# eth-cscs/COSTA

Hardware: AMD Instinct MI355X
Metric: GB/s device-resident tile pack+transpose+unpack (fp64), % HBM peak (higher is better)
Workload: dtype f64; 1 GPU; pxtran fp64 16384x16384, 256x256 blocks, op T, alpha=1 beta=0, 1x1 grid (BASELINE configs[1]); op=T, parallelism=1 rank(s), one per GPU, RCCL send/recv exchange, m=16384, n=16384, block=256, grid=1x1

## Files before the change

costa_amd/__init__.py:

```python
from __future__ import annotations

import ctypes as C
import os
import struct
from dataclasses import dataclass
from typing import Iterable, Sequence

import numpy as np

__all__ = [
    "CostaError", "lib", "FLOAT", "DOUBLE", "CFLOAT", "CDOUBLE", "INT32", "HALF", "BFLOAT16",
    "FP8_E4M3", "FP8_E5M2", "dtype_code", "element_code",
    "np_dtype", "Layout", "block_cyclic_layout", "custom_layout", "Comm", "transform",
    "transform_batch", "transform_async", "transform_batch_async", "synchronize", "transformer", "copy_and_transform", "execute_tiles", "execute_tiles_mixed",
    "convert_subtile", "TileOp", "TriOp", "TRI_OP_DTYPE", "transform_tri", "transform_tri_async",
    "execute_tiles_tri", "plan_export_tri", "tri_cut", "tri_subtile", "tri_phase_ms",
    "plan_export", "set_profiling", "get_stats", "release_caches", "TILE_OP_DTYPE",
    "ScaledOp", "SCALED_OP_DTYPE", "SCALED_F_ROWS", "transform_scaled", "execute_tiles_scaled",
    "plan_export_scaled", "scaled_subtile", "scaled_items",
]

FLOAT, DOUBLE, CFLOAT, CDOUBLE, INT32 = 0, 1, 2, 3, 4
HALF, BFLOAT16 = 5, 6
_NP = {FLOAT: np.float32, DOUBLE: np.float64, CFLOAT: np.complex64,
       CDOUBLE: np.complex128, INT32: np.int32, HALF: np.float16, BFLOAT16: np.uint16}
_TORCH = {"torch.float32": FLOAT, "torch.float64": DOUBLE, "torch.complex64": CFLOAT,
          "torch.complex128": CDOUBLE, "torch.int32": INT32, "torch.float16": HALF,
          "torch.bfloat16": BFLOAT16}

FP8_E4M3, FP8_E5M2 = 7, 8
_NP_FP8 = {FP8_E4M3: np.uint8, FP8_E5M2: np.uint8}
_TORCH_FP8 = {"torch.float8_e4m3fn": FP8_E4M3, "torch.float8_e5m2": FP8_E5M2}
_FP32_SCALARS = (HALF, BFLOAT16, FP8_E4M3, FP8_E5M2)

TILE_TRANSPOSE, TILE_CONJ, TILE_VEC_SRC, TILE_VEC_DST = 0x1, 0x2, 0x4, 0x8
SCALE_BITCOPY, SCALE_ZERO, SCALE_ALPHA, SCALE_AXPBY = 0, 1, 2, 3

TILE_OP_DTYPE = np.dtype([("src", "<u8"), ("dst", "<u8"), ("nf", "<i4"), ("ns", "<i4"),
                          ("lds", "<i4"), ("ldd", "<i4"), ("flags", "<u4"),
                          ("order", "<u4")])


TRI_LE = 0x40
TRI_OP_DTYPE = np.dtype(TILE_OP_DTYPE.descr + [("diag", "<i4"), ("pad", "<i4")])


SCALED_F_ROWS = 0x80
SCALED_OP_DTYPE = np.dtype([("op", TILE_OP_DTYPE), ("row0", "<i4"), ("col0", "<i4")])


class CostaError(RuntimeError):

# ... 139 lines not shown
        "costa_hip_synchronize": (i, [vp]),
        "costa_hip_device_count": (i, [C.POINTER(i)]),
        "costa_hip_rccl_version": (i, [C.POINTER(i)]),
        "costa_hip_copy_and_transform": (i, [i, i, i, vp, i, i, vp, i, i, i, i, vp, vp]),
        "costa_hip_execute_tiles": (i, [i, C.POINTER(TileOp), i64, vp, vp, vp, i, i]),
        "costa_hip_execute_tiles_mixed": (i, [i, i, C.POINTER(TileOp), i64, vp, vp, vp, i, i]),
        "costa_hip_convert_subtile": (i, [i, i, C.POINTER(i), C.POINTER(i)]),
        "costa_hip_transform_tri": (i, [vp, vp, c, c, i, vp, vp, vp]),
        "costa_hip_transform_tri_async": (i, [vp, vp, c, c, i, vp, vp, vp, vp]),
        "costa_hip_execute_tiles_tri": (i, [i, C.POINTER(TriOp), i64, vp, vp, vp, i, i]),
        "costa_hip_tri_cut": (i, []),
        "costa_hip_tri_phase_ms": (i, [C.POINTER(C.c_double), i]),
        "costa_hip_tri_subtile": (i, [i, C.POINTER(i), C.POINTER(i)]),
        "costa_hip_plan_export_tri": (i, [vp, vp, c, c, i, vp, vp, i, i, C.POINTER(TriPlanInfo), vp, vp,
                                          vp, vp, vp, vp, vp, vp, vp, vp]),
        "costa_hip_transform_scaled": (i, [vp, vp, c, vp, vp, vp, vp, vp]),
        "costa_hip_transform_scaled_async": (i, [vp, vp, c, vp, vp, vp, vp, vp, vp]),
        "costa_hip_execute_tiles_scaled": (i, [i, i, C.POINTER(ScaledOp), i64, vp, vp, vp, i, vp, vp, i]),
        "costa_hip_scaled_subtile": (i, [i, i, C.POINTER(i), C.POINTER(i)]),
        "costa_hip_scaled_items": (i, [C.POINTER(i64), i]),
        "costa_hip_plan_export_scaled": (i, [vp, vp, c, vp, vp, i, i, C.POINTER(ScaledPlanInfo), vp, vp,
                                             vp, vp, vp, vp, vp, vp]),
        "costa_hip_plan_export": (i, [i, C.POINTER(vp), C.POINTER(vp), C.c_char_p, vp, vp, i, i,
                                      C.POINTER(PlanInfo), vp, vp, vp, vp, vp, vp, vp, vp]),
        "costa_hip_set_profiling": (i, [i]),
        "costa_hip_get_stats": (i, [C.POINTER(FullStats), i]),
        "costa_hip_release_caches": (i, []),
        "costa_hip_set_host_staging": (i, [i]),
        "costa_hip_set_planner": (i, [i]),
        "costa_hip_plan_export_device": (i, [i, i, C.POINTER(vp), C.POINTER(vp), C.c_char_p, vp, vp,
                                             i, i, C.POINTER(PlanInfo), vp, vp, vp, vp, vp, vp, vp,
                                             vp]),
        "costa_hip_set_list_builder": (i, [i]),
        "costa_hip_work_export": (i, [i, vp, i64, i, i, vp, i64, vp, i64, C.POINTER(i64)]),
    }
    for name, (res, args) in sig.items():
        f = getattr(L, name)
        f.restype = res
        f.argtypes = args
    _lib = L
    return L


def _check(rc: int):
    if rc != 0:
        raise CostaError(rc, lib().costa_hip_last_error().decode(errors="replace"))


def _ptr(p) -> int:
    if p is None:
        return 0
    if isinstance(p, int):
        return p
    if isinstance(p, np.ndarray):
        return p.ctypes.data
    if hasattr(p, "data_ptr"):
        return p.data_ptr()
    raise TypeError(f"cannot take the address of {type(p)}")


def _scalar_bytes(code: int, x) -> bytes:
    if code in _FP32_SCALARS:
        code = FLOAT
    if code == DOUBLE:
        return struct.pack("<d", float(x))
    if code == CDOUBLE:
# ... 460 lines not shown
    po = np.zeros(b.n_pack, TILE_OP_DTYPE)
    ls = np.zeros(info.n_local_scaled, SCALED_OP_DTYPE)
    us = np.zeros(info.n_unpack_scaled, SCALED_OP_DTYPE)
    cnt = [np.zeros(nranks, np.int64) for _ in range(4)]
    sc = np.zeros(2 * b.n_slots, _NP[code])
    _check(L.costa_hip_plan_export_scaled(*args, po.ctypes.data, ls.ctypes.data, us.ctypes.data,
                                          *[x.ctypes.data for x in cnt], sc.ctypes.data))
    return ScaledPlan(np.zeros(b.n_local, TILE_OP_DTYPE), po, np.zeros(b.n_unpack, TILE_OP_DTYPE), *cnt,
                      sc, b.send_elems, b.recv_elems, b.local_elems, ls, us)


def set_profiling(on: bool = True):
    _check(lib().costa_hip_set_profiling(int(on)))


def get_stats(reset: bool = False) -> dict:
    s = FullStats()
    _check(lib().costa_hip_get_stats(C.byref(s), int(reset)))
    return s.as_dict()


def release_caches():
    _check(lib().costa_hip_release_caches())


def set_planner(mode: int):
    _check(lib().costa_hip_set_planner(int(mode)))


def set_list_builder(mode: int):
    _check(lib().costa_hip_set_list_builder(int(mode)))


@dataclass
class WorkLists:
    ordered: np.ndarray
    work: np.ndarray
    meta: dict
    on_gpu: bool


_WORK_META = ("n_large", "n_medium", "n_skew", "n_cblock", "cblock_lds", "cb_map", "tiny_first",
              "n_tiny", "n_ordered", "n_work", "on_gpu", "flags")


def work_export(dtype, ops: np.ndarray, kind: str = "local", device=None) -> WorkLists:
    code = element_code(dtype)
    ops = np.ascontiguousarray(ops, dtype=TILE_OP_DTYPE)
    k = {"local": 0, "pack": 1, "unpack": 2}[kind]
    dev = -1 if device is None else int(device)
    meta = (C.c_int64 * 12)()
    L = lib()
    _check(L.costa_hip_work_export(code, ops.ctypes.data, ops.size, k, dev, None, 0, None, 0, meta))
    o = np.zeros(meta[8], TILE_OP_DTYPE)
    w = np.zeros(meta[9], np.uint64)
    _check(L.costa_hip_work_export(code, ops.ctypes.data, ops.size, k, dev, o.ctypes.data, o.size,
                                   w.ctypes.data, w.size, meta))
    m = dict(zip(_WORK_META, list(meta)))
    return WorkLists(o, w, m, bool(m["on_gpu"]))


def set_host_staging(mode: int):
    _check(lib().costa_hip_set_host_staging(int(mode)))


def rccl_version() -> int:
# ... 4 lines not shown
```

costa_amd/csrc/capi.cpp:

```cpp
#include "engine.hpp"

#include <hip/hip_runtime.h>

#include <costa/transform.hpp>

#include <algorithm>
#include <cctype>
#include <complex>
#include <cstring>
#include <new>

struct costa_layout_s {
    costa::engine::elayout e;
    std::vector<int> base_owners;
};
struct costa_comm_s {
    costa::engine::comm* c = nullptr;
};

namespace {
thread_local std::string g_last_error;

template <typename F>
int guarded(F&& f) {
// ... 576 lines not shown
                                 int nranks, costa_plan_info_t* info, costa_tile_op_t* local_ops,
                                 costa_tile_op_t* pack_ops, costa_tile_op_t* unpack_ops,
                                 int64_t* send_counts, int64_t* send_displs, int64_t* recv_counts,
                                 int64_t* recv_displs, void* scalars) {
    device_restore keep;
    return export_plan(
        [&](const std::vector<job>& jobs) {
            auto p = costa::engine::make_plan_device(jobs, rank, nranks, 0, device, nullptr);
            if (!p)
                throw costa::engine::error(COSTA_ERR_ARG,
                                           "costa: the device planner does not apply to these "
                                           "layouts (local blocks are not exactly the rank's grid "
                                           "cells)");
            return p;
        },
        n, A, C, trans, alpha, beta, rank, nranks, info, local_ops, pack_ops, unpack_ops,
        send_counts, send_displs, recv_counts, recv_displs, scalars);
}

int costa_hip_set_planner(int mode) {
    return guarded([&] {
        if (mode < 0 || mode > 2) throw costa::engine::error(COSTA_ERR_ARG, "mode must be 0, 1 or 2");
        costa::engine::set_planner_mode(mode);
    });
}

int costa_hip_set_list_builder(int mode) {
    return guarded([&] {
        if (mode < 0 || mode > 2) throw costa::engine::error(COSTA_ERR_ARG, "mode must be 0, 1 or 2");
        costa::engine::set_list_builder_mode(mode);
    });
}

int costa_hip_work_export(int dtype, const costa_tile_op_t* ops, int64_t n_ops, int kind, int device,
                          costa_tile_op_t* ordered, int64_t cap_ordered, uint64_t* work,
                          int64_t cap_work, int64_t* meta) {
    auto body = [&] {
        if (!meta || (n_ops > 0 && !ops) || n_ops < 0) throw costa::engine::error(COSTA_ERR_ARG, "null argument");
        if (dtype < COSTA_FLOAT || dtype > COSTA_INT32) throw costa::engine::error(COSTA_ERR_ARG, "bad dtype");
        if (kind < 0 || kind > 2) throw costa::engine::error(COSTA_ERR_ARG, "kind must be 0, 1 or 2");
        std::vector<costa_tile_op_t> in(ops, ops + n_ops), o;
        std::vector<uint64_t> w;
        costa::engine::work_split ws;
        const bool on_gpu = costa::engine::work_export(
            costa_dtype_t(dtype), in, costa::engine::list_kind(kind), device, o, w, ws);
        const int64_t m[12] = {ws.n_large, ws.n_medium, ws.n_skew, ws.n_cblock, ws.cblock_lds, ws.cb_map,
                               ws.tiny_first, ws.n_tiny, int64_t(o.size()), int64_t(w.size()), on_gpu,
                               int64_t(ws.tr_shape) | int64_t(ws.sq) << 1 | int64_t(ws.full) << 2 |
                                   int64_t(ws.med_full) << 3 | int64_t(ws.med_sq) << 4 |
                                   int64_t(ws.skew_wide) << 5};
        std::memcpy(meta, m, sizeof(m));
        if (ordered && cap_ordered >= int64_t(o.size()) && !o.empty())
            std::memcpy(ordered, o.data(), o.size() * sizeof(o[0]));
        if (work && cap_work >= int64_t(w.size()) && !w.empty()) std::memcpy(work, w.data(), w.size() * sizeof(w[0]));
    };
    return device >= 0 ? gpu_guarded(body) : guarded(body);
}

int costa_hip_set_profiling(int on) {
    costa::engine::set_profiling(on != 0);
    return COSTA_OK;
}

int costa_hip_get_stats(costa_stats_t* out, int reset) {
    return guarded([&] {
        if (!out) throw costa::engine::error(COSTA_ERR_ARG, "null argument");
// ... 159 lines not shown
```

costa_amd/csrc/engine.cpp:

```cpp
#include <exception>
#include <thread>
#include "engine.hpp"

#include <hip/hip_runtime.h>
#include <rccl/rccl.h>

#include <algorithm>
#include <numeric>
#include <chrono>
#include <cmath>
#include <cstdio>
#include <cstdlib>
#include <cstring>
#include <deque>
#include <list>
#include <map>
#include <mutex>
#include <unordered_map>

namespace costa {
namespace engine {

#define HIP_CHECK(x)                                                                   \
    do {                                                                               \
        hipError_t e_ = (x);                                                           \
        if (e_ != hipSuccess)                                                          \
            throw error(COSTA_ERR_HIP, std::string(#x " failed: ") + hipGetErrorString(e_)); \
    } while (0)
#define NCCL_CHECK(x)                                                                   \
    do {                                                                                \
        ncclResult_t r_ = (x);                                                          \
        if (r_ != ncclSuccess)                                                          \
            throw error(COSTA_ERR_NCCL, std::string(#x " failed: ") + ncclGetErrorString(r_)); \
    } while (0)

namespace {
costa_stats_t g_stats{};
bool g_profiling = false;
std::recursive_mutex g_mutex;
}
// ... 363 lines not shown
        pieces[i] = uint64_t(g.nfc * g.nsc);
        total += pieces[i];
    }
    std::vector<uint32_t> by_hint(n);
    for (size_t i = 0; i < n; ++i) by_hint[i] = uint32_t(i);
    std::stable_sort(by_hint.begin(), by_hint.end(),
                     [&](uint32_t x, uint32_t y) { return ops[x]->order < ops[y]->order; });
    std::vector<uint32_t> band(n);
    uint64_t cum = 0;
    for (const uint32_t i : by_hint) {
        band[i] = uint32_t(std::min<uint64_t>(nb - 1, cum * nb / std::max<uint64_t>(total, 1)));
        cum += pieces[i];
    }
    std::stable_sort(perm.begin(), perm.end(), [&](uint32_t x, uint32_t y) { return band[x] < band[y]; });
}

void sort_pairs_by_key(std::vector<std::pair<uint64_t, uint64_t>>& kv) {
    const size_t n = kv.size();
    if (n < 2) return;
    uint64_t lo = ~uint64_t(0), hi = 0;
    for (const auto& p : kv) lo = std::min(lo, p.first), hi = std::max(hi, p.first);
    std::vector<std::pair<uint64_t, uint64_t>> tmp(n);
    std::vector<uint32_t> at((size_t(1) << 16) + 1);
    const uint64_t span = hi - lo;
    for (int sh = 0; sh == 0 || (sh < 64 && (span >> sh) != 0); sh += 16) {
        std::fill(at.begin(), at.end(), 0u);
        for (const auto& p : kv) ++at[(((p.first - lo) >> sh) & 0xFFFFu) + 1];
        for (size_t d = 1; d < at.size(); ++d) at[d] += at[d - 1];
        for (const auto& p : kv) tmp[at[((p.first - lo) >> sh) & 0xFFFFu]++] = p;
        kv.swap(tmp);
    }
}

void merge_adjacent(std::vector<costa_tile_op_t>& v, int64_t E, std::vector<uint32_t>* root = nullptr) {
    std::vector<uint32_t> id(v.size());
    for (size_t i = 0; i < v.size(); ++i) id[i] = uint32_t(i);
    if (root) {
        root->resize(v.size());
        for (size_t i = 0; i < v.size(); ++i) (*root)[i] = uint32_t(i);
    }
    if (v.size() < 2) return;
    for (int pass = 0; pass < 2; ++pass) {
        std::vector<std::pair<uint64_t, uint64_t>> kv(v.size());
        for (size_t i = 0; i < v.size(); ++i) kv[i] = {v[i].src, i};
        sort_pairs_by_key(kv);
        std::vector<uint32_t> idx(v.size());
        for (size_t k = 0; k < v.size(); ++k) idx[k] = uint32_t(kv[k].second);
        int tb = 4;
        while ((size_t(1) << tb) < 2 * v.size()) ++tb;
        const size_t tmask = (size_t(1) << tb) - 1;
        std::vector<std::pair<uint64_t, uint32_t>> table(tmask + 1, {~uint64_t(0), 0u});
        auto slot_of = [&](uint64_t a) { return size_t((a * 0x9E3779B97F4A7C15ull) >> (64 - tb)); };
        for (size_t i = 0; i < v.size(); ++i) {
            size_t h = slot_of(v[i].src);
            while (table[h].first != ~uint64_t(0) && table[h].first != v[i].src) h = (h + 1) & tmask;
            if (table[h].first == ~uint64_t(0)) table[h] = {v[i].src, uint32_t(i)};
        }
        auto find_src = [&](uint64_t a) -> int64_t {
            for (size_t h = slot_of(a);; h = (h + 1) & tmask) {
                if (table[h].first == a) return int64_t(table[h].second);
                if (table[h].first == ~uint64_t(0)) return -1;
            }
        };
        std::vector<char> gone(v.size(), 0);
        for (const uint32_t i : idx) {
            if (gone[i]) continue;
            costa_tile_op_t& a = v[i];
            const bool tr = a.flags & COSTA_TILE_TRANSPOSE;
            for (;;) {
                const int64_t n = pass == 0 ? a.ns : a.nf;
                const uint64_t next_src = a.src + uint64_t(pass == 0 ? n * a.lds * E : n * E);
                const uint64_t next_dst =
                    a.dst + uint64_t(pass == 0 ? (tr ? n : n * a.ldd) * E : (tr ? n * a.ldd : n) * E);
                const int64_t nx = find_src(next_src);
                if (nx < 0 || gone[nx] || uint32_t(nx) == i) break;
                const costa_tile_op_t& b = v[size_t(nx)];
                const uint32_t vec = COSTA_TILE_VEC_SRC | COSTA_TILE_VEC_DST;
                const bool same = b.dst == next_dst && (b.flags & ~vec) == (a.flags & ~vec) && b.lds == a.lds &&
                                  b.ldd == a.ldd && (pass == 0 ? b.nf == a.nf : b.ns == a.ns);
                const int64_t total = n + (pass == 0 ? b.ns : b.nf);
                if (!same || total > (int64_t(1) << 30)) break;
                (pass == 0 ? a.ns : a.nf) = int32_t(total);
                if (!a.order) a.order = b.order;
                gone[nx] = 1;
                if (root) (*root)[id[nx]] = id[i];
            }
        }
        size_t o = 0;
        for (size_t i = 0; i < v.size(); ++i)
            if (!gone[i]) {
                id[o] = id[i];
                v[o++] = v[i];
            }
        v.resize(o);
        id.resize(o);
    }
    if (root)
        for (size_t i = 0; i < root->size(); ++i) {
            uint32_t r = (*root)[i];
            while ((*root)[r] != r) r = (*root)[r];
            (*root)[i] = r;
        }
}

std::vector<costa_tile_op_t> merge_filled(const std::vector<costa_tile_op_t>& cand, int64_t E, int bf, int bs) {
    std::vector<costa_tile_op_t> v = cand;
    std::vector<uint32_t> root;
    merge_adjacent(v, E, &root);
    if (v.size() == cand.size()) return v;
    std::vector<costa_tile_op_t> out;
    out.reserve(cand.size());
    std::vector<char> keep(cand.size(), 0);
    std::vector<uint32_t> count(cand.size(), 0);
    for (size_t i = 0; i < cand.size(); ++i) ++count[root[i]];
    size_t k = 0;
    for (size_t i = 0; i < cand.size(); ++i) {
        if (root[i] != i) continue;
        const costa_tile_op_t& m = v[k++];
        keep[i] = count[i] == 1 || (2 * int64_t(m.nf) >= bf && 2 * int64_t(m.ns) >= bs);
        if (keep[i]) out.push_back(m);
    }
    for (size_t i = 0; i < cand.size(); ++i)
        if (!keep[root[i]]) out.push_back(cand[i]);
    return out;
}

bool few_strides(const std::vector<costa_tile_op_t>& ops) {
    int32_t seen[16];
    int k = 0;
// ... 388 lines not shown
            continue;
        }
        const uint64_t row_bytes = uint64_t(op.ldd) * uint64_t(E);
        const int64_t p = 64 / int64_t(std::gcd(row_bytes % 64 == 0 ? uint64_t(64) : row_bytes % 64, uint64_t(64)));
        const uint32_t keep_vs = E == 4 ? (op.flags & COSTA_TILE_VEC_SRC) : 0u;
        for (int64_t r = 0; r < std::min<int64_t>(p, op.ns); ++r) {
            costa_tile_op_t part = op;
            part.src = op.src + uint64_t(r * int64_t(op.lds) * E);
            part.dst = op.dst + uint64_t(r * int64_t(op.ldd) * E);
            part.ns = int32_t((op.ns - r + p - 1) / p);
            part.lds = int32_t(int64_t(op.lds) * p);
            part.ldd = int32_t(int64_t(op.ldd) * p);
            const int64_t eps = int64_t(part.dst % 64) / E;
            const int64_t h = eps > 0 ? std::min<int64_t>(op.nf, G - eps) : 0;
            if (h > 0) {
                costa_tile_op_t head = part;
                head.nf = int32_t(h);
                head.flags = (op.flags & ~vec_bits) | vec_flags(head.src, head.lds, head.dst, head.ldd, E) | keep_vs;
                out.push_back(head);
            }
            if (h < op.nf) {
                costa_tile_op_t body = part;
                body.src += uint64_t(h * E);
                body.dst += uint64_t(h * E);
                body.nf = int32_t(op.nf - h);
                body.flags = (op.flags & ~vec_bits) | vec_flags(body.src, body.lds, body.dst, body.ldd, E) | keep_vs;
                out.push_back(body);
            }
        }
    }
    return true;
}

work_split build_work(costa_dtype_t dtype, const std::vector<costa_tile_op_t>& ops_in,
                      std::vector<costa_tile_op_t>& ordered, std::vector<uint64_t>& work,
                      list_kind kind, device_section* dev, bool dst_order) {
    const bool pack_list = kind == list_pack, local = kind == list_local;
    static const int mis_env = [] {
        const char* s = tuning_env("COSTA_MISALIGNED_VEC");
        return s ? std::atoi(s) : -1;
    }();
    const int mis = mis_env >= 0 ? mis_env : dtype_size(dtype) == 4 ? 2 : 0;
    const wave_knobs& kn0 = knobs();
    static const bool trace = std::getenv("COSTA_PLAN_TRACE") != nullptr;
    const auto bw0 = std::chrono::steady_clock::now();
    double bw_t[4] = {0, 0, 0, 0};
    double sub_t[3] = {0, 0, 0};
    auto lap = [&](int k) {
        if (!trace) return;
        const double t = std::chrono::duration<double, std::milli>(std::chrono::steady_clock::now() - bw0).count();
        bw_t[k] = t;
    };
    auto mark = [&](int k) {
        if (trace) sub_t[k] = std::chrono::duration<double, std::milli>(std::chrono::steady_clock::now() - bw0).count();
    };
    std::vector<costa_tile_op_t> ops_merged;
    const std::vector<costa_tile_op_t>* ops_src = &ops_in;
    if (kn0.merge && ops_in.size() > 1 && few_strides(ops_in)) {
        shape_dims sh0;
        tile_shapes(dtype, any_transpose(ops_in), &sh0);
        const int64_t half_large = kn0.merge == 1 ? int64_t(sh0.cf) * sh0.cs / 2 : INT64_MAX;
        std::vector<costa_tile_op_t> cand;
        for (const auto& op : ops_in)
            (int64_t(op.nf) * op.ns < half_large ? cand : ops_merged).push_back(op);
        const size_t n_cand0 = cand.size();
        cand = merge_filled(cand, int64_t(dtype_size(dtype)), sh0.cf, sh0.cs);
// ... 127 lines not shown
    }
    mark(2);
    std::vector<uint32_t> shaped[3];
    std::vector<costa_tile_op_t> skew_ops;
    for (size_t li = 0; li < ops.size(); ++li) {
        const int c = cls[li] == 1 && n_med < kMinMediumOps ? 2 : cls[li];
        if (c < 2) shaped[c].push_back(uint32_t(li));
        else if (c == 2) wave_ops.push_back(&ops[li]);
        else if (c == 4) skew_ops.push_back(ops[li]);
    }
    merge_adjacent(skew_ops, E);
    for (size_t i = 0; i < skew_ops.size(); ++i) shaped[2].push_back(uint32_t(i));
    bool skew_wide = false;
    for (const auto& op : skew_ops)
        skew_wide = skew_wide || (E == 4 && (op.src % 16 != 0 || (uint64_t(op.lds) * uint64_t(E)) % 16 != 0));
    const int64_t skew_group = kn.skew_xcd >= 0 ? kn.skew_xcd : skew_wide ? kSkewWideGroup : 0;
    int64_t n_work[3] = {0, 0, 0};
    for (int c = 0; c < 3; ++c) {
        const int bf = c == 2 ? (skew_wide ? sh.bf_kw : sh.bf_k) : c ? (med_sq ? sh.bf_s : sh.bf_m) : sq ? sh.bf_q : sh.bf;
        const int bs = c == 2 ? (skew_wide ? sh.bs_kw : sh.bs_k) : c ? (med_sq ? sh.bs_s : sh.bs_m) : sq ? sh.bs_q : sh.bs;
        const std::vector<uint32_t>& sel = shaped[c];
        const std::vector<costa_tile_op_t>& src_ops = c == 2 ? skew_ops : ops;
        std::vector<uint32_t> sperm(sel.size());
        for (size_t i = 0; i < sel.size(); ++i) sperm[i] = uint32_t(i);
        if (kn.large_sort >= 1 && !sel.empty()) {
            bool hints = true;
            for (uint32_t li : sel) hints = hints && src_ops[li].order != 0;
            if (hints)
                std::stable_sort(sperm.begin(), sperm.end(), [&](uint32_t x, uint32_t y) {
                    return src_ops[sel[x]].order < src_ops[sel[y]].order;
                });
        }
        const size_t op0 = ordered.size(), w0 = work.size();
        for (const uint32_t k : sperm) {
            const costa_tile_op_t& op = src_ops[sel[k]];
            const uint64_t i = ordered.size();
            if (i > 0xFFFFFFFFull) throw error(COSTA_ERR_ARG, "costa: too many tiles in one list");
            ordered.push_back(op);
            const uint64_t n = uint64_t((op.nf + bf - 1) / bf) * uint64_t((op.ns + bs - 1) / bs);
            if (n > 0xFFFFFFFFull) throw error(COSTA_ERR_ARG, "costa: tile too large");
            for (uint64_t q = 0; q < n; ++q) work.push_back((i << 32) | q);
        }
        bool by_address = kn.large_sort == 2 || dst_order;
        if (kn.large_sort == 3 && !dst_order) {
            by_address = (E == 4 || E == 8 || (E == 16 && c == 0 && sq)) && ordered.size() > op0;
            for (size_t i = op0; i < ordered.size(); ++i)
                by_address = by_address && (ordered[i].flags & COSTA_TILE_TRANSPOSE);
        }
        if (by_address && work.size() - w0 > 1) {
            std::vector<std::pair<uint64_t, uint64_t>> key(work.size() - w0);
            for (size_t x = 0; x < key.size(); ++x) {
                const uint64_t wx = work[w0 + x];
                const costa_tile_op_t& op = ordered[size_t(wx >> 32)];
                const uint64_t q = wx & 0xFFFFFFFFull, nbf = uint64_t((op.nf + bf - 1) / bf);
                const int64_t f0 = int64_t(q % nbf) * bf, s0 = int64_t(q / nbf) * bs;
                const bool tr = op.flags & COSTA_TILE_TRANSPOSE;
                key[x] = {op.dst + uint64_t((tr ? f0 * op.ldd + s0 : s0 * op.ldd + f0) * E), wx};
            }
            int64_t panel = kn.panel_rows;
            const int64_t ld0 = ordered[size_t(key[0].second >> 32)].ldd;
            bool one_ld = true;
            for (size_t i = op0; i < ordered.size() && one_ld; ++i) one_ld = ordered[i].ldd == ld0;
            if (panel == 0)
                panel = ld0 * E > kPanelBytes && dtype != COSTA_CFLOAT ? kPanelBytes / E : -1;
            if (panel >= (int64_t(1) << 24)) panel = -1;
            if (panel > 0 && one_ld) {
                uint64_t lo = ~uint64_t(0), hi = 0;
                for (const auto& k : key) {
                    lo = std::min(lo, k.first);
                    hi = std::max(hi, k.first);
                }
                const uint64_t ld = uint64_t(ld0), last = (hi - lo) / uint64_t(E);
                const bool fits = last / ld < (uint64_t(1) << 24) && ld / uint64_t(panel) < (uint64_t(1) << 16);
                if (fits) {
                    for (auto& k : key) {
                        const uint64_t e = (k.first - lo) / uint64_t(E);
                        const uint64_t row = e % ld, col = e / ld;
                        k.first = ((row / uint64_t(panel)) << 48) | (col << 24) | (row % uint64_t(panel));
                    }
                }
            }
            sort_pairs_by_key(key);
// ... 375 lines not shown
constexpr size_t kDevicePlanBlocks = 4096;
constexpr size_t kColdDevicePlanBlocks = 100000;
bool g_device_planner_warm = false;
}

int planner_mode() {
    if (g_planner < 0) {
        const char* s = std::getenv("COSTA_PLANNER");
        g_planner = s ? std::max(0, std::min(2, std::atoi(s))) : 1;
    }
    return g_planner;
}

void set_planner_mode(int mode) {
    std::lock_guard<std::recursive_mutex> lk(g_mutex);
    g_planner = mode;
}

namespace {
int g_list_builder = -1;
}

int list_builder_mode() {
    if (g_list_builder < 0) {
        const char* s = std::getenv("COSTA_LIST_BUILDER");
        g_list_builder = s ? std::max(0, std::min(2, std::atoi(s))) : 1;
    }
    return g_list_builder;
}

void set_list_builder_mode(int mode) {
    std::lock_guard<std::recursive_mutex> lk(g_mutex);
    g_list_builder = mode;
}

namespace {
template <typename X>
void upload_list(dbuf& d, const std::vector<X>& h, const X* sec, size_t at, size_t n, hipStream_t s) {
    if (!sec || n == 0) return d.upload(h, s);
    const size_t total = h.size() + n;
    d.reserve(total * sizeof(X));
    X* p = static_cast<X*>(d.p);
    if (at) HIP_CHECK(hipMemcpyAsync(p, h.data(), at * sizeof(X), hipMemcpyHostToDevice, s));
    HIP_CHECK(hipMemcpyAsync(p + at, sec, n * sizeof(X), hipMemcpyDeviceToDevice, s));
    if (h.size() > at)
        HIP_CHECK(hipMemcpyAsync(p + at + n, h.data() + at, (h.size() - at) * sizeof(X), hipMemcpyHostToDevice, s));
}
}

bool work_export(costa_dtype_t dtype, const std::vector<costa_tile_op_t>& ops, list_kind kind, int device,
                 std::vector<costa_tile_op_t>& ordered, std::vector<uint64_t>& work, work_split& w) {
    std::lock_guard<std::recursive_mutex> lk(g_mutex);
    if (device < 0) {
        w = build_work(dtype, ops, ordered, work, kind);
        return false;
    }
    device_ctx& dc = ctx(device);
    device_section sec;
    sec.device = device;
    sec.stream = dc.main;
    sec.force = true;
    w = build_work(dtype, ops, ordered, work, kind, &sec);
    if (!sec.n_ordered) return false;
    std::vector<costa_tile_op_t> o(sec.n_ordered);
    std::vector<uint64_t> k(sec.n_work);
    HIP_CHECK(hipMemcpyAsync(o.data(), sec.d_ordered, o.size() * sizeof(o[0]), hipMemcpyDeviceToHost, dc.main));
// ... 842 lines not shown
```

costa_amd/csrc/engine.hpp:

```cpp
#pragma once

#include <costa/layout.hpp>
#include <costa_hip.h>

#include <array>
#include <cstdint>
#include <functional>
#include <memory>
#include <string>
#include <vector>

namespace costa {
namespace engine {

size_t dtype_size(costa_dtype_t t);
bool dtype_is_complex(costa_dtype_t t);
bool dtype_is_half(costa_dtype_t t);
costa_dtype_t compute_dtype(costa_dtype_t src, costa_dtype_t dst);
bool half_pair(costa_dtype_t src, costa_dtype_t dst);
bool dtype_is_fp8(costa_dtype_t t);
bool fp8_pair(costa_dtype_t src, costa_dtype_t dst);
costa_dtype_t plan_pkg_dtype(costa_dtype_t src, costa_dtype_t dst);

struct eblock {
// ... 244 lines not shown
    int bf_kw = 0, bs_kw = 0;
};
void tile_shapes(costa_dtype_t dtype, bool transposing_list, shape_dims* out);
struct work_split {
    int64_t n_large = 0, n_medium = 0, tiny_first = 0, n_tiny = 0;
    int64_t n_skew = 0;
    int64_t n_cblock = 0;
    int64_t cblock_lds = 0;
    int cb_map = 0;
    bool tr_shape = false;
    bool sq = false;
    bool full = false;
    bool med_full = false;
    bool med_sq = false;
    bool skew_wide = false;
    int64_t n_items() const { return n_large + n_medium + n_skew + n_cblock + n_tiny; }
};
enum list_kind { list_local, list_pack, list_unpack };
struct device_section {
    int device = -1;
    void* stream = nullptr;
    bool force = false;
    std::shared_ptr<void> mem;
    costa_tile_op_t* d_ordered = nullptr;
    uint64_t* d_work = nullptr;
    size_t at_ordered = 0, n_ordered = 0, at_work = 0, n_work = 0;
};
work_split build_work(costa_dtype_t dtype, const std::vector<costa_tile_op_t>& ops,
                      std::vector<costa_tile_op_t>& ordered, std::vector<uint64_t>& work,
                      list_kind kind = list_local, device_section* dev = nullptr, bool dst_order = false);
constexpr size_t kDeviceGroupsMin = 16384;
int list_builder_mode();
void set_list_builder_mode(int mode);
int64_t cblock_groups_device(int64_t E, int64_t budget, uint32_t vec_bits, int bands_env,
                             const std::vector<costa_tile_op_t>& ops, const std::vector<uint32_t>& wave,
                             size_t base_at, device_section& sec, std::vector<char>& taken,
                             int64_t& lds, int& map);
bool work_export(costa_dtype_t dtype, const std::vector<costa_tile_op_t>& ops, list_kind kind,
                 int device, std::vector<costa_tile_op_t>& ordered, std::vector<uint64_t>& work,
                 work_split& w);
launch_args make_launch(const work_split& w, const void* d_ordered, const void* d_work,
                        const char* src_base, char* dst_base, const void* d_scalars, bool transpose,
                        bool axpby);

struct host_pipeline;
bool host_pipeline_accepts(costa_dtype_t dtype, const std::vector<costa_tile_op_t>& pack_ops);
std::shared_ptr<host_pipeline> make_host_pipeline(costa_dtype_t dtype,
                                                  const std::vector<costa_tile_op_t>& pack_ops,
                                                  const std::vector<costa_tile_op_t>& local_ops,
                                                  const std::vector<costa_tile_op_t>& unpack_ops,
                                                  const std::vector<int>& pack_round,
                                                  const std::vector<int>& unpack_round, int rounds);
size_t host_pipeline_groups(const host_pipeline& hp);
void run_host_pipeline(host_pipeline& hp, int device, void* compute_stream, void* exchange_stream,
                       char* send_buf, char* recv_buf,
                       const std::function<void(void*, int)>& exchange, const void* d_scalars);
void exchange_round_of_ops(const struct plan& p, int rounds, std::vector<int>& pack_round,
                           std::vector<int>& unpack_round);
void exchange_round_of_tri(const struct plan& p, int rounds, std::vector<int>& unpack_tri_round);
void release_host_rings();
int host_staging_mode();
void set_host_staging_mode(int mode);

struct error : std::runtime_error {
    int code;
    error(int c, const std::string& m) : std::runtime_error(m), code(c) {}
// ... 10 lines not shown
```

include/costa_hip.h:

```cpp
#ifndef COSTA_HIP_H
#define COSTA_HIP_H

#include <stddef.h>
#include <stdint.h>

#ifdef __cplusplus
extern "C" {
#endif

#define COSTA_OK 0
#define COSTA_ERR_ARG 1
#define COSTA_ERR_HIP 2
#define COSTA_ERR_NCCL 3
#define COSTA_ERR_INTERNAL 4

typedef enum {
    COSTA_FLOAT = 0,
    COSTA_DOUBLE = 1,
    COSTA_CFLOAT = 2,
    COSTA_CDOUBLE = 3,
    COSTA_INT32 = 4,
    COSTA_HALF = 5,
    COSTA_BFLOAT16 = 6,
    COSTA_FP8_E4M3 = 7,
// ... 171 lines not shown
typedef struct {
    double pack_ms, local_ms, unpack_ms, exchange_ms, h2d_ms, d2h_ms;
    int64_t pack_launches, local_launches, unpack_launches;
    int64_t pack_bytes, local_bytes, unpack_bytes;
    int64_t transforms;
    int64_t plan_hits, plan_misses;
    int64_t host_groups;
    int64_t device_plans;
    double plan_ms;
    int64_t host_direct;
    int64_t host_direct_groups;
    int64_t tile_items, skew_items, cblock_items, tiny_items;
    int64_t device_lists;
    int64_t fused_pieces;
    int64_t convert_items;
    int64_t tri_items;
} costa_stats_t;
int costa_hip_tri_phase_ms(double* ms, int reset);
int costa_hip_set_profiling(int on);
int costa_hip_get_stats(costa_stats_t* out, int reset);
int costa_hip_release_caches(void);

int costa_hip_set_host_staging(int mode);

int costa_hip_set_planner(int mode);
int costa_hip_plan_export_device(int device, int n, const costa_layout_t* A, const costa_layout_t* C,
                                 const char* trans, const void* alpha, const void* beta, int rank,
                                 int nranks, costa_plan_info_t* info, costa_tile_op_t* local_ops,
                                 costa_tile_op_t* pack_ops, costa_tile_op_t* unpack_ops,
                                 int64_t* send_counts, int64_t* send_displs, int64_t* recv_counts,
                                 int64_t* recv_displs, void* scalars);

int costa_hip_set_list_builder(int mode);
int costa_hip_work_export(int dtype, const costa_tile_op_t* ops, int64_t n_ops, int kind, int device,
                          costa_tile_op_t* ordered, int64_t cap_ordered, uint64_t* work,
                          int64_t cap_work, int64_t* meta);

#ifdef __cplusplus
}
#endif
#endif
```

Before: 6203 GB/s.

## Add fast paths for tile merging and address-ordered work item generation

Adds a lattice-based merge that recognises grid-structured runs of adjacent tile ops and collapses them without the general sort-based pairwise merge. It also adds a direct generator that emits work items in destination-address order for small op counts, skipping the key sort. Both sit behind a default-on global switch with counters. The target is host-side planning cost, which matters only if planning is inside the timed region, and the merge logic is intricate enough that a wrong merge could produce incorrect tiles.

```diff
diff --git a/costa_amd/__init__.py b/costa_amd/__init__.py
--- a/costa_amd/__init__.py
+++ b/costa_amd/__init__.py
@@ -18,6 +18,7 @@
     "plan_export", "set_profiling", "get_stats", "release_caches", "TILE_OP_DTYPE",
     "ScaledOp", "SCALED_OP_DTYPE", "SCALED_F_ROWS", "transform_scaled", "execute_tiles_scaled",
     "plan_export_scaled", "scaled_subtile", "scaled_items",
+    "set_work_fastpath", "work_fastpath_counts",
 ]
 
 FLOAT, DOUBLE, CFLOAT, CDOUBLE, INT32 = 0, 1, 2, 3, 4
@@ -223,6 +224,8 @@
                                              i, i, C.POINTER(PlanInfo), vp, vp, vp, vp, vp, vp, vp,
                                              vp]),
         "costa_hip_set_list_builder": (i, [i]),
+        "costa_hip_set_work_fastpath": (i, [i]),
+        "costa_hip_work_fastpath_counts": (i, [C.POINTER(i64), i]),
         "costa_hip_work_export": (i, [i, vp, i64, i, i, vp, i64, vp, i64, C.POINTER(i64)]),
     }
     for name, (res, args) in sig.items():
@@ -749,6 +752,16 @@
     _check(lib().costa_hip_set_list_builder(int(mode)))
 
 
+def set_work_fastpath(on: bool = True):
+    _check(lib().costa_hip_set_work_fastpath(int(bool(on))))
+
+
+def work_fastpath_counts(reset: bool = False) -> dict:
+    c = (C.c_int64 * 5)()
+    _check(lib().costa_hip_work_fastpath_counts(c, int(reset)))
+    return dict(zip(("merge_fast", "merge_general", "order_fast", "order_general", "general_joined"), list(c)))
+
+
 @dataclass
 class WorkLists:
     ordered: np.ndarray
diff --git a/costa_amd/csrc/capi.cpp b/costa_amd/csrc/capi.cpp
--- a/costa_amd/csrc/capi.cpp
+++ b/costa_amd/csrc/capi.cpp
@@ -632,6 +632,17 @@
     });
 }
 
+int costa_hip_set_work_fastpath(int on) {
+    return guarded([&] { costa::engine::set_work_fastpath(on != 0); });
+}
+
+int costa_hip_work_fastpath_counts(int64_t* counts, int reset) {
+    return guarded([&] {
+        if (!counts) throw costa::engine::error(COSTA_ERR_ARG, "null argument");
+        costa::engine::work_fastpath_counts(counts, reset != 0);
+    });
+}
+
 int costa_hip_work_export(int dtype, const costa_tile_op_t* ops, int64_t n_ops, int kind, int device,
                           costa_tile_op_t* ordered, int64_t cap_ordered, uint64_t* work,
                           int64_t cap_work, int64_t* meta) {
diff --git a/costa_amd/csrc/engine.cpp b/costa_amd/csrc/engine.cpp
--- a/costa_amd/csrc/engine.cpp
+++ b/costa_amd/csrc/engine.cpp
@@ -6,6 +6,7 @@
 #include <rccl/rccl.h>
 
 #include <algorithm>
+#include <atomic>
 #include <numeric>
 #include <chrono>
 #include <cmath>
@@ -435,6 +436,167 @@
     }
 }
 
+std::atomic<int> g_work_fastpath{1};
+std::atomic<int64_t> g_fast_count[5];
+
+bool lattice_merge(std::vector<costa_tile_op_t>& v, int64_t E, std::vector<uint32_t>* root) {
+    const size_t n = v.size();
+    const uint32_t vec = COSTA_TILE_VEC_SRC | COSTA_TILE_VEC_DST;
+    const int64_t cap = int64_t(1) << 30;
+    auto cont = [&](const costa_tile_op_t& a, const costa_tile_op_t& b, bool along_f) {
+        if ((a.flags & ~vec) != (b.flags & ~vec) || a.lds != b.lds || a.ldd != b.ldd) return false;
+        const bool tr = a.flags & COSTA_TILE_TRANSPOSE;
+        if (along_f)
+            return b.ns == a.ns && b.src == a.src + uint64_t(int64_t(a.nf) * E) &&
+                   b.dst == a.dst + uint64_t((tr ? int64_t(a.nf) * a.ldd : int64_t(a.nf)) * E);
+        return b.nf == a.nf && b.src == a.src + uint64_t(int64_t(a.ns) * a.lds * E) &&
+               b.dst == a.dst + uint64_t((tr ? int64_t(a.ns) : int64_t(a.ns) * a.ldd) * E);
+    };
+    struct run {
+        size_t at, A, B;
+        bool inner_f;
+        int64_t NF, NS;
+        uint64_t src_hi;
+        size_t nfc() const { return inner_f ? B : A; }
+        size_t nsc() const { return inner_f ? A : B; }
+        size_t index(size_t i, size_t j) const { return inner_f ? at + j * B + i : at + i * B + j; }
+    };
+    std::vector<run> runs;
+    for (size_t k = 0; k < n;) {
+        if (2 * (runs.size() + 1) > n) return false;
+        const costa_tile_op_t& o = v[k];
+        if (o.nf <= 0 || o.ns <= 0 || o.lds <= 0 || o.ldd <= 0 || o.nf > o.lds) return false;
+        run r{k, 1, 1, false, 0, 0, 0};
+        const bool f = k + 1 < n && cont(o, v[k + 1], true);
+        if (f || (k + 1 < n && cont(o, v[k + 1], false))) {
+            r.inner_f = f;
+            r.B = 2;
+            while (k + r.B < n && cont(v[k + r.B - 1], v[k + r.B], f)) ++r.B;
+            for (;; ++r.A) {
+                const size_t h = k + r.A * r.B;
+                if (h + r.B > n || !cont(v[h - r.B], v[h], !f)) break;
+                bool ok = true;
+                for (size_t b = 1; b < r.B && ok; ++b)
+                    ok = cont(v[h + b - 1], v[h + b], f) &&
+                         (f ? v[h + b].nf == v[k + b].nf : v[h + b].ns == v[k + b].ns);
+                if (!ok) break;
+            }
+        }
+        bool positive = true;
+        for (size_t i = 0; i < r.nfc(); ++i) r.NF += v[r.index(i, 0)].nf, positive = positive && v[r.index(i, 0)].nf > 0;
+        for (size_t j = 0; j < r.nsc(); ++j) r.NS += v[r.index(0, j)].ns, positive = positive && v[r.index(0, j)].ns > 0;
+        if (!positive || r.NF > cap || r.NS > cap || r.NF > o.lds) return false;
+        k += r.A * r.B;
+        r.src_hi = v[k - 1].src;
+        runs.push_back(r);
+    }
+    const size_t m = runs.size();
+    auto f_at = [&](const run& r, size_t i) { return int64_t((v[r.index(i, 0)].src - v[r.at].src) / uint64_t(E)); };
+    auto s_at = [&](const run& r, size_t j) {
+        return int64_t((v[r.index(0, j)].src - v[r.at].src) / (uint64_t(E) * uint64_t(v[r.at].lds)));
+    };
+    int64_t budget = 16 * int64_t(n) + 65536;
+    if (m > 1) {
+        budget -= int64_t(m) * int64_t(m);
+        if (budget < 0) return false;
+    }
+    for (size_t x = 0; x < m; ++x)
+        for (size_t y = x + 1; y < m; ++y) {
+            const run& X = v[runs[x].at].src <= v[runs[y].at].src ? runs[x] : runs[y];
+            const run& Y = &X == &runs[x] ? runs[y] : runs[x];
+            const uint64_t x0 = v[X.at].src, y0 = v[Y.at].src;
+            if (X.src_hi < y0) continue;
+            const int64_t ld = v[X.at].lds;
+            if (v[Y.at].lds != ld || (y0 - x0) % uint64_t(E) != 0) return false;
+            const int64_t d = int64_t((y0 - x0) / uint64_t(E));
+            const int64_t xf = f_at(X, X.nfc() - 1), yf = f_at(Y, Y.nfc() - 1);
+            int64_t r0 = d / ld, c0 = d % ld;
+            if (c0 + yf >= ld) {
+                r0 += 1, c0 -= ld;
+                if (std::max(xf, c0 + yf) - c0 >= ld) return false;
+            }
+            if (c0 > xf || c0 + yf < 0 || r0 > s_at(X, X.nsc() - 1)) continue;
+            budget -= int64_t(X.nfc() + Y.nfc() + X.nsc() + Y.nsc());
+            if (budget < 0) return false;
+            bool cols = false, rows = false;
+            for (size_t i = 0, j = 0; !cols && i < X.nfc() && j < Y.nfc();) {
+                const int64_t a = f_at(X, i), b = c0 + f_at(Y, j);
+                cols = a == b;
+                a < b ? ++i : ++j;
+            }
+            for (size_t i = 0, j = 0; cols && !rows && i < X.nsc() && j < Y.nsc();) {
+                const int64_t a = s_at(X, i), b = r0 + s_at(Y, j);
+                rows = a == b;
+                a < b ? ++i : ++j;
+            }
+            if (cols && rows) return false;
+        }
+    auto find = [&](uint64_t p) -> int64_t {
+        for (const run& Y : runs) {
+            const uint64_t y0 = v[Y.at].src;
+            if (p < y0 || p > Y.src_hi || (p - y0) % uint64_t(E) != 0) continue;
+            const int64_t d = int64_t((p - y0) / uint64_t(E)), ld = v[Y.at].lds, s = d / ld, fo = d % ld;
+            size_t lo = 0, hi = Y.nfc();
+            while (lo + 1 < hi) {
+                const size_t mid = (lo + hi) / 2;
+                (f_at(Y, mid) <= fo ? lo : hi) = mid;
+            }
+            if (f_at(Y, lo) != fo) continue;
+            const size_t i = lo;
+            lo = 0, hi = Y.nsc();
+            while (lo + 1 < hi) {
+                const size_t mid = (lo + hi) / 2;
+                (s_at(Y, mid) <= s ? lo : hi) = mid;
+            }
+            if (s_at(Y, lo) == s) return int64_t(Y.index(i, lo));
+        }
+        return -1;
+    };
+    for (size_t x = 0; m > 1 && x < m; ++x) {
+        const run& X = runs[x];
+        const costa_tile_op_t& o = v[X.at];
+        const bool tr = o.flags & COSTA_TILE_TRANSPOSE;
+        budget -= int64_t(X.nfc() + 1) * int64_t(m);
+        if (budget < 0) return false;
+        for (size_t i = 0; i < X.nfc(); ++i) {
+            const costa_tile_op_t& h = v[X.index(i, 0)];
+            const int64_t nx = find(h.src + uint64_t(X.NS * o.lds * E));
+            if (nx < 0) continue;
+            const costa_tile_op_t& b = v[size_t(nx)];
+            if (b.dst == h.dst + uint64_t((tr ? X.NS : X.NS * o.ldd) * E) && (b.flags & ~vec) == (o.flags & ~vec) &&
+                b.lds == o.lds && b.ldd == o.ldd && b.nf == h.nf)
+                return false;
+        }
+        const int64_t nx = find(o.src + uint64_t(X.NF * E));
+        if (nx < 0) continue;
+        const costa_tile_op_t& b = v[size_t(nx)];
+        const run* Y = nullptr;
+        for (const run& r : runs)
+            if (size_t(nx) >= r.at && size_t(nx) < r.at + r.A * r.B) Y = &r;
+        bool head = false;
+        for (size_t i = 0; i < Y->nfc() && !head; ++i) head = Y->index(i, 0) == size_t(nx);
+        if (head && b.dst == o.dst + uint64_t((tr ? X.NF * o.ldd : X.NF) * E) &&
+            (b.flags & ~vec) == (o.flags & ~vec) && b.lds == o.lds && b.ldd == o.ldd && Y->NS == X.NS)
+            return false;
+    }
+    if (root) {
+        root->resize(n);
+        for (const run& r : runs)
+            for (size_t i = r.at; i < r.at + r.A * r.B; ++i) (*root)[i] = uint32_t(r.at);
+    }
+    for (size_t x = 0; x < m; ++x) {
+        const run& r = runs[x];
+        costa_tile_op_t mo = v[r.at];
+        mo.nf = int32_t(r.NF);
+        mo.ns = int32_t(r.NS);
+        for (size_t i = 0; !mo.order && i < r.nfc(); ++i)
+            for (size_t j = 0; !mo.order && j < r.nsc(); ++j) mo.order = v[r.index(i, j)].order;
+        v[x] = mo;
+    }
+    v.resize(m);
+    return true;
+}
+
 void merge_adjacent(std::vector<costa_tile_op_t>& v, int64_t E, std::vector<uint32_t>* root = nullptr) {
     std::vector<uint32_t> id(v.size());
     for (size_t i = 0; i < v.size(); ++i) id[i] = uint32_t(i);
@@ -443,6 +605,10 @@
         for (size_t i = 0; i < v.size(); ++i) (*root)[i] = uint32_t(i);
     }
     if (v.size() < 2) return;
+    const size_t root_size = v.size();
+    const bool took = g_work_fastpath.load() && lattice_merge(v, E, root);
+    ++g_fast_count[took ? 0 : 1];
+    if (took) return;
     for (int pass = 0; pass < 2; ++pass) {
         std::vector<std::pair<uint64_t, uint64_t>> kv(v.size());
         for (size_t i = 0; i < v.size(); ++i) kv[i] = {v[i].src, i};
@@ -498,6 +664,7 @@
         v.resize(o);
         id.resize(o);
     }
+    if (v.size() < root_size) ++g_fast_count[4];
     if (root)
         for (size_t i = 0; i < root->size(); ++i) {
             uint32_t r = (*root)[i];
@@ -952,6 +1119,69 @@
     return true;
 }
 
+static bool items_by_address(costa_dtype_t dtype, const std::vector<costa_tile_op_t>& ordered, size_t op0, int bf,
+                             int bs, int64_t E, int64_t panel, uint64_t* out) {
+    constexpr size_t kMaxOps = 64;
+    const size_t n_ops = ordered.size() - op0;
+    if (n_ops == 0 || n_ops > kMaxOps) return false;
+    struct span {
+        uint64_t lo, hi;
+        size_t i;
+    };
+    span sp[kMaxOps];
+    const int64_t ld0 = ordered[op0].ldd;
+    bool one_ld = true;
+    uint64_t lo = ~uint64_t(0), hi = 0;
+    for (size_t k = 0; k < n_ops; ++k) {
+        const costa_tile_op_t& op = ordered[op0 + k];
+        const bool tr = op.flags & COSTA_TILE_TRANSPOSE;
+        const int64_t nbf = (op.nf + bf - 1) / bf, nbs = (op.ns + bs - 1) / bs;
+        if (nbf < 1 || nbs < 1) return false;
+        const int64_t in_col = tr ? (nbs - 1) * bs : (nbf - 1) * bf, cols = tr ? (nbf - 1) * bf : (nbs - 1) * bs;
+        if (in_col >= op.ldd) return false;
+        sp[k] = {op.dst, op.dst + uint64_t((cols * op.ldd + in_col) * E), op0 + k};
+        one_ld = one_ld && op.ldd == ld0;
+        lo = std::min(lo, sp[k].lo);
+        hi = std::max(hi, sp[k].hi);
+    }
+    if (panel == 0) panel = ld0 * E > kPanelBytes && dtype != COSTA_CFLOAT ? kPanelBytes / E : -1;
+    if (panel >= (int64_t(1) << 24) || !one_ld) panel = -1;
+    if (panel > 0) {
+        const uint64_t ld = uint64_t(ld0), last = (hi - lo) / uint64_t(E);
+        if (!(last / ld < (uint64_t(1) << 24) && ld / uint64_t(panel) < (uint64_t(1) << 16))) panel = -1;
+    }
+    if (panel > 0) {
+        if (n_ops != 1) return false;
+        const costa_tile_op_t& op = ordered[op0];
+        const bool tr = op.flags & COSTA_TILE_TRANSPOSE;
+        const int64_t nbf = (op.nf + bf - 1) / bf, nbs = (op.ns + bs - 1) / bs;
+        const int64_t n_in = tr ? nbs : nbf, n_cols = tr ? nbf : nbs, step = tr ? bs : bf;
+        const uint64_t head = uint64_t(op0) << 32;
+        for (int64_t r0 = 0, r1; r0 < n_in; r0 = r1) {
+            for (r1 = r0 + 1; r1 < n_in && r1 * step / panel == r0 * step / panel;) ++r1;
+            for (int64_t cc = 0; cc < n_cols; ++cc)
+                for (int64_t r = r0; r < r1; ++r) *out++ = head | uint64_t(tr ? r * nbf + cc : cc * nbf + r);
+        }
+        return true;
+    }
+    std::sort(sp, sp + n_ops, [](const span& a, const span& b) { return a.lo < b.lo; });
+    for (size_t k = 0; k + 1 < n_ops; ++k)
+        if (sp[k].hi >= sp[k + 1].lo) return false;
+    for (size_t k = 0; k < n_ops; ++k) {
+        const costa_tile_op_t& op = ordered[sp[k].i];
+        const bool tr = op.flags & COSTA_TILE_TRANSPOSE;
+        const int64_t nbf = (op.nf + bf - 1) / bf, nbs = (op.ns + bs - 1) / bs;
+        const uint64_t head = uint64_t(sp[k].i) << 32;
+        if (tr) {
+            for (int64_t fi = 0; fi < nbf; ++fi)
+                for (int64_t sj = 0; sj < nbs; ++sj) *out++ = head | uint64_t(sj * nbf + fi);
+        } else {
+            for (int64_t q = 0; q < nbf * nbs; ++q) *out++ = head | uint64_t(q);
+        }
+    }
+    return true;
+}
+
 work_split build_work(costa_dtype_t dtype, const std::vector<costa_tile_op_t>& ops_in,
                       std::vector<costa_tile_op_t>& ordered, std::vector<uint64_t>& work,
                       list_kind kind, device_section* dev, bool dst_order) {
@@ -1145,14 +1375,14 @@
                 });
         }
         const size_t op0 = ordered.size(), w0 = work.size();
+        size_t n_sub = 0;
         for (const uint32_t k : sperm) {
             const costa_tile_op_t& op = src_ops[sel[k]];
-            const uint64_t i = ordered.size();
-            if (i > 0xFFFFFFFFull) throw error(COSTA_ERR_ARG, "costa: too many tiles in one list");
+            if (ordered.size() > 0xFFFFFFFFull) throw error(COSTA_ERR_ARG, "costa: too many tiles in one list");
             ordered.push_back(op);
             const uint64_t n = uint64_t((op.nf + bf - 1) / bf) * uint64_t((op.ns + bs - 1) / bs);
             if (n > 0xFFFFFFFFull) throw error(COSTA_ERR_ARG, "costa: tile too large");
-            for (uint64_t q = 0; q < n; ++q) work.push_back((i << 32) | q);
+            n_sub += size_t(n);
         }
         bool by_address = kn.large_sort == 2 || dst_order;
         if (kn.large_sort == 3 && !dst_order) {
@@ -1160,7 +1390,23 @@
             for (size_t i = op0; i < ordered.size(); ++i)
                 by_address = by_address && (ordered[i].flags & COSTA_TILE_TRANSPOSE);
         }
-        if (by_address && work.size() - w0 > 1) {
+        by_address = by_address && n_sub > 1;
+        work.resize(w0 + n_sub);
+        bool placed = false;
+        if (by_address) {
+            if (g_work_fastpath.load())
+                placed = items_by_address(dtype, ordered, op0, bf, bs, E, kn.panel_rows, work.data() + w0);
+            ++g_fast_count[placed ? 2 : 3];
+        }
+        if (!placed) {
+            uint64_t* out = work.data() + w0;
+            for (size_t i = op0; i < ordered.size(); ++i) {
+                const costa_tile_op_t& op = ordered[i];
+                const uint64_t n = uint64_t((op.nf + bf - 1) / bf) * uint64_t((op.ns + bs - 1) / bs);
+                for (uint64_t q = 0; q < n; ++q) *out++ = (uint64_t(i) << 32) | q;
+            }
+        }
+        if (by_address && !placed) {
             std::vector<std::pair<uint64_t, uint64_t>> key(work.size() - w0);
             for (size_t x = 0; x < key.size(); ++x) {
                 const uint64_t wx = work[w0 + x];
@@ -1602,6 +1848,12 @@
 void set_list_builder_mode(int mode) {
     std::lock_guard<std::recursive_mutex> lk(g_mutex);
     g_list_builder = mode;
+}
+
+void set_work_fastpath(bool on) { g_work_fastpath.store(on ? 1 : 0); }
+bool work_fastpath() { return g_work_fastpath.load() != 0; }
+void work_fastpath_counts(int64_t out[5], bool reset) {
+    for (int i = 0; i < 5; ++i) out[i] = reset ? g_fast_count[i].exchange(0) : g_fast_count[i].load();
 }
 
 namespace {
diff --git a/costa_amd/csrc/engine.hpp b/costa_amd/csrc/engine.hpp
--- a/costa_amd/csrc/engine.hpp
+++ b/costa_amd/csrc/engine.hpp
@@ -300,6 +300,9 @@
 constexpr size_t kDeviceGroupsMin = 16384;
 int list_builder_mode();
 void set_list_builder_mode(int mode);
+void set_work_fastpath(bool on);
+bool work_fastpath();
+void work_fastpath_counts(int64_t out[5], bool reset);
 int64_t cblock_groups_device(int64_t E, int64_t budget, uint32_t vec_bits, int bands_env,
                              const std::vector<costa_tile_op_t>& ops, const std::vector<uint32_t>& wave,
                              size_t base_at, device_section& sec, std::vector<char>& taken,
diff --git a/include/costa_hip.h b/include/costa_hip.h
--- a/include/costa_hip.h
+++ b/include/costa_hip.h
@@ -227,6 +227,8 @@
                                  int64_t* recv_displs, void* scalars);
 
 int costa_hip_set_list_builder(int mode);
+int costa_hip_set_work_fastpath(int on);
+int costa_hip_work_fastpath_counts(int64_t* counts, int reset);
 int costa_hip_work_export(int dtype, const costa_tile_op_t* ops, int64_t n_ops, int kind, int device,
                           costa_tile_op_t* ordered, int64_t cap_ordered, uint64_t* work,
                           int64_t cap_work, int64_t* meta);
```

Result: no change. 6206 GB/s (median of 5 runs) (+0.0%).
